# LiChaiUSTC/Speech-enhancement-based-on-a-maximum-likelihood-criterion

Hardware: AMD Instinct MI355X
Metric: training frames/sec (128-frame minibatch) (higher is better)
Workload: dtype f32

## Files before the change

include/mlggd.h:

```cpp
#ifndef MLGGD_H
#define MLGGD_H

#include <stddef.h>
#include <stdint.h>

#ifdef __cplusplus
extern "C" {
#endif

#define MLGGD_MAXLAYER 10
#define MLGGD_MAXCACHEFRAME 200000
#define MLGGD_UNIQUE_ID_BYTES 128
#define MLGGD_MAX_BETAS 32

enum {
    MLGGD_OK = 0,
    MLGGD_ERR_ARG = 1,
    MLGGD_ERR_DEVICE = 2,
    MLGGD_ERR_COMM = 3,
    MLGGD_ERR_STATE = 4
};

typedef struct mlggd_engine *mlggd_handle;

// ... 117 lines not shown

int mlggd_profile_select(mlggd_handle h, const char *kernel_class, int layer, int max_launches);
int mlggd_profile_stride(mlggd_handle h, int every_nth_step);
int mlggd_profile_read(mlggd_handle h, float *mean_usec, int *launches);
int mlggd_profile_overhead(mlggd_handle h, float *usec);
int mlggd_kernel_work(mlggd_handle h, const char *kernel_class, int layer, double *flops, double *bytes);
int mlggd_dw_launches_per_step(mlggd_handle h, int *launches);
int mlggd_dp_mode(mlggd_handle h, int *mode);
int mlggd_debug_fake_world(mlggd_handle h, int world_size, int mode);
int mlggd_debug_keep_ranks(mlggd_handle h, int on);
int mlggd_debug_rank_tensor(mlggd_handle h, const char *name, int layer, int rank, float *dst, size_t count);
int mlggd_debug_plan_count(mlggd_handle h, int *plans);

int mlggd_debug_out_slabs(mlggd_handle h, int *slabs);
int mlggd_debug_gemm_plan(mlggd_handle h, int layer, int *fwd_waves, int *dx_waves);

int mlggd_debug_math(mlggd_handle h, const char *fn, const float *x, float y, float *out, size_t n);

int mlggd_debug_stamp_select(mlggd_handle h, const char *kernel_class, int layer);
int mlggd_debug_stamp_read(mlggd_handle h, long long *out , int cap_blocks, int *blocks);

#ifdef __cplusplus
}
#endif
#endif
```

speech-enhancement-based-on-a-maximum-likelihood-criterion_amd/__init__.py:

```python
import collections
import ctypes as C
import os
import subprocess

import numpy as np

_HERE = os.path.dirname(os.path.abspath(__file__))
_CSRC = os.path.join(_HERE, "csrc")
LIB_PATH = os.path.join(_CSRC, "libmlggd.so")
MAXLAYER = 10
UNIQUE_ID_BYTES = 128

_fp = C.POINTER(C.c_float)
_fpp = C.POINTER(_fp)


class MlggdError(RuntimeError):
    pass


class _Config(C.Structure):
    _fields_ = [
        ("struct_size", C.c_int32), ("random_seed", C.c_int32), ("device", C.c_int32),
        ("numlayers", C.c_int32), ("layersizes", C.c_int32 * MAXLAYER), ("bunchsize", C.c_int32),
# ... 4 lines not shown
    ]


EXPORTS = [
    "mlggd_create", "mlggd_destroy", "mlggd_last_error", "mlggd_device_count", "mlggd_train_chunk",
    "mlggd_load_chunk", "mlggd_train_resident", "mlggd_sync", "mlggd_cv_sqerr", "mlggd_cv_abserr",
    "mlggd_cv_loglik", "mlggd_cv_all", "mlggd_forward", "mlggd_get_weights", "mlggd_set_weights",
    "mlggd_get_scalefactor", "mlggd_set_scalefactor", "mlggd_set_lrate", "mlggd_gamma",
    "mlggd_debug_tensor", "mlggd_comm_unique_id", "mlggd_comm_init", "mlggd_last_train_ms",
    "mlggd_profile_select", "mlggd_profile_stride", "mlggd_profile_read", "mlggd_profile_overhead",
    "mlggd_kernel_work", "mlggd_dw_launches_per_step", "mlggd_dp_mode", "mlggd_debug_fake_world",
    "mlggd_debug_stamp_select", "mlggd_debug_stamp_read",
    "mlggd_load_frames", "mlggd_train_frames", "mlggd_train_frames_async", "mlggd_cv_all_frames", "mlggd_forward_frames",
    "mlggd_alloc_pinned", "mlggd_alloc_pinned_on", "mlggd_free_pinned", "mlggd_set_cv_device_reduce",
    "mlggd_comm_info", "mlggd_debug_plan_count", "mlggd_debug_math", "mlggd_debug_out_slabs", "mlggd_debug_gemm_plan",
    "mlggd_debug_keep_ranks", "mlggd_debug_rank_tensor",
    "mlggd_wave_to_lps", "mlggd_lps_to_wave", "mlggd_enhance_wave",
    "mlggd_enhance_waves_layout", "mlggd_enhance_waves",
    "mlggd_score_waves", "mlggd_enhance_waves_scored",
    "mlggd_stoi_layout", "mlggd_stoi_waves", "mlggd_enhance_waves_scored_stoi",
    "mlggd_live_layout", "mlggd_live_open", "mlggd_live_push", "mlggd_live_received", "mlggd_live_close",
    "mlggd_error_stats", "mlggd_error_stats_frames", "mlggd_ggd_fit",
]
MAX_BETAS = 32

_lib = None


def build(force=False):
    srcs = [os.path.join(_CSRC, f) for f in ("engine.hip", "kernels.hip.h", "kernels64.hip.h", "spectral.hip.h", "score.hip.h", "live.hip.h",
# ... 42 lines not shown
    L.mlggd_profile_select.argtypes = [C.c_void_p, C.c_char_p, C.c_int, C.c_int]
    L.mlggd_profile_stride.argtypes = [C.c_void_p, C.c_int]
    L.mlggd_profile_read.argtypes = [C.c_void_p, _fp, C.POINTER(C.c_int)]
    L.mlggd_profile_overhead.argtypes = [C.c_void_p, _fp]
    L.mlggd_kernel_work.argtypes = [C.c_void_p, C.c_char_p, C.c_int, C.POINTER(C.c_double),
                                    C.POINTER(C.c_double)]
    L.mlggd_dw_launches_per_step.argtypes = [C.c_void_p, C.POINTER(C.c_int)]
    L.mlggd_dp_mode.argtypes = [C.c_void_p, C.POINTER(C.c_int)]
    L.mlggd_debug_fake_world.argtypes = [C.c_void_p, C.c_int, C.c_int]
    L.mlggd_debug_keep_ranks.argtypes = [C.c_void_p, C.c_int]
    L.mlggd_debug_rank_tensor.argtypes = [C.c_void_p, C.c_char_p, C.c_int, C.c_int, _fp, C.c_size_t]
    L.mlggd_comm_info.argtypes = [C.c_void_p, C.POINTER(C.c_int), C.POINTER(C.c_int)]
    L.mlggd_debug_plan_count.argtypes = [C.c_void_p, C.POINTER(C.c_int)]
    L.mlggd_debug_out_slabs.argtypes = [C.c_void_p, C.POINTER(C.c_int)]
    L.mlggd_debug_gemm_plan.argtypes = [C.c_void_p, C.c_int, C.POINTER(C.c_int), C.POINTER(C.c_int)]
    L.mlggd_debug_math.argtypes = [C.c_void_p, C.c_char_p, _fp, C.c_float, _fp, C.c_size_t]
    L.mlggd_debug_stamp_select.argtypes = [C.c_void_p, C.c_char_p, C.c_int]
    L.mlggd_debug_stamp_read.argtypes = [C.c_void_p, C.POINTER(C.c_longlong), C.c_int, C.POINTER(C.c_int)]
    _ip = C.POINTER(C.c_int32)
    L.mlggd_load_frames.argtypes = [C.c_void_p, C.c_int, C.c_int, _fp, _fp, C.c_int, _ip, C.c_int]
    L.mlggd_train_frames.argtypes = [C.c_void_p, C.c_int, C.c_int, _fp, _fp, C.c_int, _ip, C.c_int, C.POINTER(C.c_int)]
    L.mlggd_train_frames_async.argtypes = L.mlggd_train_frames.argtypes
    L.mlggd_cv_all_frames.argtypes = [C.c_void_p, C.c_int, C.c_int, _fp, _fp, C.c_int, _ip, C.c_int, _fp, _fp, _fp]
    L.mlggd_forward_frames.argtypes = [C.c_void_p, C.c_int, C.c_int, _fp, C.c_int, _ip, _fp]
    L.mlggd_alloc_pinned.argtypes = [C.c_size_t, C.POINTER(C.c_void_p)]
    L.mlggd_free_pinned.argtypes = [C.c_void_p]
    _sp = C.POINTER(C.c_int16)
    L.mlggd_wave_to_lps.argtypes = [C.c_int, C.c_int, C.c_int, _sp, C.POINTER(C.c_int), _fp]
    L.mlggd_lps_to_wave.argtypes = [C.c_int, C.c_int, C.c_int, _sp, C.c_int, _fp, _sp, _fp]
    L.mlggd_enhance_wave.argtypes = [C.c_void_p, C.c_int, C.c_int, _fp, _fp, C.c_int, _sp, _sp, _fp, C.POINTER(C.c_int)]
# ... 614 lines not shown
        return n.value

    def out_slabs(self):
        n = C.c_int(0)
        _check(load().mlggd_debug_out_slabs(self._h, C.byref(n)))
        return n.value

    def gemm_plan(self):
        out = []
        for l in range(1, len(self.layersizes)):
            f, d = C.c_int(0), C.c_int(0)
            _check(load().mlggd_debug_gemm_plan(self._h, l, C.byref(f), C.byref(d)))
            out.append((f.value, d.value))
        return out

    def comm_info(self):
        n, r = C.c_int(0), C.c_int(-1)
        _check(load().mlggd_comm_info(self._h, C.byref(n), C.byref(r)))
        return n.value, r.value

    def debug_math(self, fn, x, y=0.0):
        x = _f32(x).ravel()
        out = np.empty_like(x)
        _check(load().mlggd_debug_math(self._h, fn.encode(), _p(x), float(y), _p(out), x.size))
        return out

    def plan_count(self):
        n = C.c_int(0)
        _check(load().mlggd_debug_plan_count(self._h, C.byref(n)))
        return n.value
# ... 46 lines not shown
```

speech-enhancement-based-on-a-maximum-likelihood-criterion_amd/csrc/engine.hip:

```cpp
#include <hip/hip_runtime.h>
#include <hip/hip_ext.h>

#include <dlfcn.h>
#include <math.h>
#include <stdarg.h>
#include <stdio.h>
#include <stdlib.h>
#include <string.h>

#include <functional>
#include <mutex>
#include <string>
#include <vector>

#include "../../include/mlggd.h"
#include "kernels.hip.h"
#include "spectral.hip.h"
#include "score.hip.h"
#include "stoi.hip.h"
#include "stoi_rule.h"
#include "live.hip.h"
#include "live_rule.h"
#include "errstats.hip.h"

// ... 172 lines not shown
        WsBuf wave, lps, X, blk, out_i, out_f, lps_den, norm, frame_off, out_off, wave_off, utt_of;
        WsBuf clean, Xc, fstat, sframes, scores;
        WsBuf stoi_utt, stoi_x, stoi_f, stoi_i, stoi_res;
        std::vector<int32_t> h_frame_off, h_utt_of;
        std::vector<long long> h_out_off, h_wave_off;
        std::vector<float> h_norm;
        std::vector<float> h_scores;
        std::vector<StoiUtt> h_stoi_utt;
        std::vector<float> h_stoi;
        int lookup_table = 0;
    } ww;
    int live_groups = 0;
    bool indexed = false;
    int fdim = 0, toff = 0, raw_frames = 0;
    unsigned step_counter = 0;
    int fwd_pipe = 4, dx_pipe = 4;
    int tile64 = 1, n_cus = 256;
    int fwd_nw = 4, dx_nw = 4, dw_tile = 1, dw_persist = 1, dwp_per_cu = 2, dw_merge = 1, loss_fuse = 1, tile_map = 0, stage_ahead = 1;

    int world = 1, rank = 0;
    int dp_mode = 0;
    int shard_rows[MLGGD_MAXLAYER] = {0};
    int dp_a2a = 0;
    std::vector<float *> Ysrc[MLGGD_MAXLAYER];
    hipEvent_t ev_W[MLGGD_MAXLAYER] = {0}, ev_dw_done = nullptr;
    bool ev_W_pending[MLGGD_MAXLAYER] = {false};
    bool fake_world = false;
    float *Yall[MLGGD_MAXLAYER] = {0}, *dEdXall[MLGGD_MAXLAYER] = {0};
    bool keep_ranks = false;
    std::vector<float *> snap_x, snap_out, snap_y[MLGGD_MAXLAYER], snap_dedx[MLGGD_MAXLAYER];
    hipEvent_t ev_ready = nullptr, ev_gathered = nullptr;
// ... 223 lines not shown
    a.fdim = e->fdim;
    a.rows_out = rows_out;
    a.yblk = e->dp_a2a ? e->shard_rows[1] * 64 : 0;
    return a;
}
static int stage_blocks(const mlggd_engine *e) { return (e->lsp[0] / 32) * (e->Bp / 32); }
static float *in_bunch_other(mlggd_engine *e) {
    return e->in_bunch == e->in_bunch_buf[0] ? e->in_bunch_buf[1] : e->in_bunch_buf[0];
}

static bool tile64_ok(const mlggd_engine *e, int units_p) {
    if (e->tile64 == 0 || units_p % 64 != 0 || e->Bp % 64 != 0) return false;
    return e->tile64 == 2 || (long)(units_p / 64) * (e->Bp / 64) >= e->n_cus;
}
static bool fwd64_used(const mlggd_engine *e, int l) {
    if (e->fwd_pipe != 4 || e->fwd_nw != 4 || !tile64_ok(e, e->lsp[l])) return false;
    return l != e->L - 1 || e->S_out == 1;
}
static bool dx64_used(const mlggd_engine *e, int l) {
    return l >= 2 && e->dx_pipe == 4 && e->dx_nw == 4 && tile64_ok(e, e->lsp[l - 1]);
}

static int run_transpose(mlggd_engine *e, const Bunch &bn, int frames) {
    ProfScope ps(e, KC_TRANSPOSE, 0);
    hipLaunchKernelGGL(k_transpose_in, dim3(stage_blocks(e)), dim3(256), 0, e->stream,
                       stage_args(e, bn, frames, e->in_bunch));
    return launch_check("k_transpose_in");
}

static int wait_weight_gathers(mlggd_engine *e, int l_lo, int l_hi) {
    for (int l = l_lo; l <= l_hi; l++)
        if (e->ev_W_pending[l]) {
            HIPCHK(hipStreamWaitEvent(e->stream, e->ev_W[l], 0));
            e->ev_W_pending[l] = false;
        }
// ... 43 lines not shown
        const int Kp = e->lsp[l - 1], Np = e->lsp[l], n_tiles = Np / 32;
        CHK(wait_weight_gathers(e, l, l));
        if (cvscale) {
            const float keep = 1.0f - ((l == 1) ? e->cfg.visible_omit : e->cfg.hid_omit);
            hipLaunchKernelGGL(k_scale, dim3(1024), dim3(256), 0, e->stream, e->W[l], (size_t)Kp * Np, keep);
        }
        {
            if (((gather_flags & GATHER_HIDDEN_EACH) && l < e->L - 1) || ((gather_flags & GATHER_HIDDEN) && l == e->L - 2))
                gather_arm(e);
            ProfScope ps(e, KC_FWD, l);
            FwdArgs fa = fwd_args(e, l, e->Y[l]);
            if (fwd64_used(e, l)) {
                fa.n_tiles = Np / 64;
                fa.b_tiles = e->Bp / 64;
                fa.b_shift = log2_or_minus1(fa.b_tiles);
                const size_t lds = t64_lds_floats() * sizeof(float);
                if (l != e->L - 1) {
                    CHK(ensure_lds(e, k_fwd64<FWD_SIGMOID>, lds));
                    launch_timed(e, k_fwd64<FWD_SIGMOID>, dim3(fa.n_tiles * fa.b_tiles), dim3(256), lds, e->stream, fa);
                } else {
                    CHK(ensure_lds(e, k_fwd64<FWD_SLAB>, lds));
                    launch_timed(e, k_fwd64<FWD_SLAB>, dim3(fa.n_tiles * fa.b_tiles), dim3(256), lds, e->stream, fa);
                }
            } else if (l != e->L - 1) {
                long long *st = stamps_for(e, KC_FWD, l, n_tiles * b_tiles);
#define LAUNCH_FWD(NW, PIPE)                                                                                \
    {                                                                                                       \
        const size_t lds = fwd_lds_floats<NW, PIPE>() * sizeof(float);                                      \
        CHK(ensure_lds(e, k_fwd<FWD_SIGMOID, NW, PIPE>, lds));                                              \
        launch_timed(e, k_fwd<FWD_SIGMOID, NW, PIPE>, dim3(n_tiles * b_tiles), dim3(64 * NW), lds, e->stream, fa, st); \
    }
                if (e->fwd_nw == 16) LAUNCH_FWD(16, 0)
                else if (e->fwd_nw == 8 && e->fwd_pipe == 4) LAUNCH_FWD(8, 4)
                else if (e->fwd_nw == 8 && e->fwd_pipe) LAUNCH_FWD(8, 1)
                else if (e->fwd_nw == 8) LAUNCH_FWD(8, 0)
                else if (e->fwd_pipe == 4) LAUNCH_FWD(4, 4)
                else if (e->fwd_pipe) LAUNCH_FWD(4, 1)
                else LAUNCH_FWD(4, 0)
#undef LAUNCH_FWD
            } else {
                const int nwg = n_tiles * b_tiles * e->S_out;
                if (e->fwd_pipe == 4) {
                    const size_t lds = fwd_lds_floats<4, 4>() * sizeof(float);
                    CHK(ensure_lds(e, k_fwd<FWD_SLAB, 4, 4>, lds));
                    launch_timed(e, k_fwd<FWD_SLAB, 4, 4>, dim3(nwg), dim3(256), lds, e->stream, fa, (long long *)nullptr);
                } else {
                    const size_t lds = fwd_lds_floats<4, 1>() * sizeof(float);
                    launch_timed(e, k_fwd<FWD_SLAB, 4, 1>, dim3(nwg), dim3(256), lds, e->stream, fa, (long long *)nullptr);
                }
            }
        }
        CHK(launch_check("k_fwd"));
        if (cvscale) {
            const float keep = 1.0f - ((l == 1) ? e->cfg.visible_omit : e->cfg.hid_omit);
            hipLaunchKernelGGL(k_scale, dim3(1024), dim3(256), 0, e->stream, e->W[l], (size_t)Kp * Np, 1.0f / keep);
        }
        if (drop && l != e->L - 1) CHK(run_dropout(e, l, nullptr));
        if ((gather_flags & GATHER_HIDDEN_EACH) && l < e->L - 1) {
            CHK(gather_begin_armed(e));
            CHK(exchange_y(e, l, e->Y[l], nullptr));
            CHK(gather_end(e));
        }
// ... 451 lines not shown
    hipLaunchKernelGGL(k_loss_grad, dim3(n_loss), dim3(256), lds_grad, e->stream, e->eT, e->pT, colsum_in, B, e->D, e->Dp, Bp,
                       e->cfg.shapefactor, ML, nf, inv_n, e->scalefactor, e->dEdXt[L - 1], e->dEdX[L - 1], b_tiles);
    return launch_check("k_loss_grad");
}

static int run_dx(mlggd_engine *e, int l) {
    const int Kp = e->lsp[l - 1], b_tiles = e->Bp / 32;
    ProfScope ps(e, KC_DX, l);
    DxArgs xa = dx_args(e, l);
    if (dx64_used(e, l)) {
        xa.k_tiles = Kp / 64;
        xa.b_tiles = e->Bp / 64;
        xa.b_shift = log2_or_minus1(xa.b_tiles);
        const size_t lds = t64_lds_floats() * sizeof(float);
        CHK(ensure_lds(e, k_dx64, lds));
        launch_timed(e, k_dx64, dim3(xa.k_tiles * xa.b_tiles), dim3(256), lds, e->stream, xa);
        return launch_check("k_dx64");
    }
    long long *st = stamps_for(e, KC_DX, l, (Kp / 32) * b_tiles);
#define LAUNCH_DX(NW, PIPE)                                                                                  \
    {                                                                                                        \
        const size_t lds = dx_lds_floats<NW, PIPE>() * sizeof(float);                                        \
        CHK(ensure_lds(e, k_dx<NW, PIPE>, lds));                                                             \
        launch_timed(e, k_dx<NW, PIPE>, dim3((Kp / 32) * b_tiles), dim3(64 * NW), lds, e->stream, xa, st);      \
    }
    const bool dma = e->dx_pipe == 4 && (Kp / 32) * b_tiles <= 256;
    if (e->dx_nw == 8 && e->dx_pipe) LAUNCH_DX(8, 1)
    else if (e->dx_nw == 8) LAUNCH_DX(8, 0)
    else if (dma) LAUNCH_DX(4, 4)
    else if (e->dx_pipe) LAUNCH_DX(4, 1)
    else LAUNCH_DX(4, 0)
#undef LAUNCH_DX
    return launch_check("k_dx");
}

static int launch_dw_layer(mlggd_engine *e, int l, const float *in_rows, bool fused, float nf, hipStream_t st) {
    const int Kp = e->lsp[l - 1], Np = e->lsp[l];
    const long tiles128 = (long)((Kp + 127) / 128) * ((Np + 127) / 128);
    const bool big = e->dw_tile == 0 ? tiles128 >= 192 : e->dw_tile == 2;
    ProfScope ps(e, KC_DW, l, st);
    if (dwp_usable(e)) return launch_dwp(e, dwp_jobs(e, l, l, in_rows, nf), fused, st, l);
    if (big) return launch_dw<2>(e, l, in_rows, fused, nf, st);
    return launch_dw<1>(e, l, in_rows, fused, nf, st);
// ... 349 lines not shown
    e->device = cfg->device;
    for (int i = 0; i < e->L; i++) {
        e->ls[i] = cfg->layersizes[i];
        e->lsp[i] = ceil32(cfg->layersizes[i]);
    }
    e->B = cfg->bunchsize;
    e->Bp = ceil32(e->B);
    e->K0 = e->ls[0];
    e->D = e->ls[e->L - 1];
    e->Dp = e->lsp[e->L - 1];
    if (const char *v = getenv("MLGGD_FWD_NW")) e->fwd_nw = atoi(v);
    if (const char *v = getenv("MLGGD_WAVES_LOOKUP")) e->ww.lookup_table = !strcmp(v, "table");
    if (const char *v = getenv("MLGGD_DX_NW")) e->dx_nw = atoi(v);
    if (const char *v = getenv("MLGGD_FWD_PIPE")) e->fwd_pipe = atoi(v);
    if (const char *v = getenv("MLGGD_DX_PIPE")) e->dx_pipe = atoi(v);
    if (const char *v = getenv("MLGGD_DW_TILE")) e->dw_tile = atoi(v);
    if (const char *v = getenv("MLGGD_TWO_STREAMS")) e->two_streams = atoi(v);
    if (const char *v = getenv("MLGGD_DW_PERSIST")) e->dw_persist = atoi(v);
    if (const char *v = getenv("MLGGD_DWP_PER_CU")) e->dwp_per_cu = atoi(v);
    if (const char *v = getenv("MLGGD_DW_MERGE")) e->dw_merge = atoi(v);
    if (const char *v = getenv("MLGGD_LOSS_FUSE")) e->loss_fuse = atoi(v);
    if (const char *v = getenv("MLGGD_TILE_MAP")) e->tile_map = atoi(v);
    if (const char *v = getenv("MLGGD_STAGE_AHEAD")) e->stage_ahead = atoi(v);
    if (const char *v = getenv("MLGGD_CV_DEVICE")) e->cv_device = atoi(v) ? 1 : 0;
    if (const char *v = getenv("MLGGD_TILE64")) e->tile64 = atoi(v);
    *out = e;

    roctx_load();
    HIPCHK(hipSetDevice(e->device));
    {
// ... 943 lines not shown
    }
    if (nranks) *nranks = n;
    if (rank) *rank = r;
    return MLGGD_OK;
}
int mlggd_debug_plan_count(mlggd_handle e, int *plans) {
    if (!e || !plans) return fail(MLGGD_ERR_ARG, "NULL argument");
    *plans = (int)e->dwp_tables.size();
    return MLGGD_OK;
}
int mlggd_debug_gemm_plan(mlggd_handle e, int layer, int *fwd_waves, int *dx_waves) {
    if (!e || !fwd_waves || !dx_waves) return fail(MLGGD_ERR_ARG, "NULL argument");
    if (layer < 1 || layer >= e->L) return fail(MLGGD_ERR_ARG, "layer %d not in 1..%d", layer, e->L - 1);
    *fwd_waves = fwd64_used(e, layer) ? 1 : e->fwd_nw;
    *dx_waves = dx64_used(e, layer) ? 1 : e->dx_nw;
    return MLGGD_OK;
}
int mlggd_debug_out_slabs(mlggd_handle e, int *slabs) {
    if (!e || !slabs) return fail(MLGGD_ERR_ARG, "NULL argument");
    *slabs = e->S_out;
    return MLGGD_OK;
}
int mlggd_dp_mode(mlggd_handle e, int *mode) {
    if (!e || !mode) return fail(MLGGD_ERR_ARG, "NULL argument");
    *mode = (e->comm || e->fake_world) ? (e->dp_a2a ? 4 : 1 + e->dp_mode) : 0;
    return MLGGD_OK;
}

int mlggd_debug_math(mlggd_handle e, const char *fn, const float *x, float y, float *out, size_t n) {
    if (!e || !fn || (n > 0 && (!x || !out))) return fail(MLGGD_ERR_ARG, "NULL argument");
// ... 1230 lines not shown
```

speech-enhancement-based-on-a-maximum-likelihood-criterion_amd/csrc/kernels.hip.h:

```cpp
#pragma once
#include <hip/hip_runtime.h>

typedef float f32x16 __attribute__((ext_vector_type(16)));
typedef float f32x2 __attribute__((ext_vector_type(2)));

__device__ __forceinline__ f32x16 mfma32(float a, float b, f32x16 c) {
    return __builtin_amdgcn_mfma_f32_32x32x2f32(a, b, c, 0, 0, 0);
}
__device__ __forceinline__ int acc_row(int r, int lane) { return (r & 3) + 8 * (r >> 2) + 4 * (lane >> 5); }

__device__ __forceinline__ void divmod_by(int x, int d, int shift, int &q, int &r) {
    if (shift >= 0) {
        q = x >> shift;
        r = x & (d - 1);
    } else {
        q = (int)((unsigned)x / (unsigned)d);
        r = x - q * d;
    }
}
__device__ __forceinline__ void tile_of_block(int id, int u_tiles, int b_tiles, int b_shift, int &ut, int &bt, int map = 0) {
    if ((u_tiles & 7) == 0 && map != 2) {
        const int xcd = id & 7, slot = id >> 3;
        int q;
        divmod_by(slot, b_tiles, b_shift, q, bt);
// ... 144 lines not shown
}

enum { FWD_SIGMOID = 0, FWD_SLAB = 1 };

struct FwdArgs {
    const float *W, *Yt_in, *bias;
    float *Yt_out, *Y_out, *slab;
    int Kp, Np, Bp, N, n_tiles, b_tiles, S, map;
    int b_shift, s_shift;
    int yblk;
};
__device__ __forceinline__ size_t y_blocked_base(int u0, int yblk, int Bp) {
    const int blk = (int)((unsigned)u0 / (unsigned)yblk);
    return (size_t)blk * Bp * yblk + (u0 - blk * yblk);
}
template <int NW, int PIPE> constexpr int fwd_lds_floats() { return NW * (PIPE == 4 ? 4096 : 2048) + 32 * 36; }

template <int MODE, int NW, int PIPE = 1>
__device__ __forceinline__ void fwd_body(const FwdArgs &A, const int bid, float *smem, long long *stamps) {
    const float *__restrict__ W = A.W, *__restrict__ Yt_in = A.Yt_in, *__restrict__ bias = A.bias;
    float *__restrict__ Yt_out = A.Yt_out, *__restrict__ Y_out = A.Y_out, *__restrict__ slab = A.slab;
    const int Kp = A.Kp, Np = A.Np, Bp = A.Bp, N = A.N, n_tiles = A.n_tiles, b_tiles = A.b_tiles, S = A.S;
    float(*tileT)[36] = reinterpret_cast<float(*)[36]>(smem + NW * (PIPE == 4 ? 4096 : 2048));
    stamp(stamps, 0, bid);
    stamp_clk(stamps, 4, bid);
    const int tid = threadIdx.x, lane = tid & 63, wave = wave_id();
    const int i = lane & 31, h = lane >> 5;
    int id = bid, s = 0;
    if (MODE == FWD_SLAB) divmod_by(bid, S, A.s_shift, id, s);
    int nt, bt;
    tile_of_block(id, n_tiles, b_tiles, A.b_shift, nt, bt, A.map);
    const int n0 = nt * 32, b0 = bt * 32;

    const int P = Kp >> 1;
    const int slot = s * NW + wave, nslots = S * NW;
    int p0, p1;
    if (MODE == FWD_SLAB) {
        p0 = (int)((unsigned)(P * slot) / (unsigned)nslots);
// ... 3 lines not shown
        p1 = (int)((unsigned)(P * (wave + 1)) / (unsigned)NW);
    }
    const int npairs = p1 - p0;
    const int nch = (npairs + 15) >> 4;

    const rsrc_t rW = make_rsrc(W, (size_t)Kp * Np * 4), rY = make_rsrc(Yt_in, (size_t)Kp * Bp * 4);
    const int r8 = lane >> 3, c4 = lane & 7;
    const int voW = (r8 * Np + n0 + 4 * c4) * 4, voY = (r8 * Bp + b0 + 4 * c4) * 4;
    float *stg = smem + wave * 2048;
    float *wdst = stg + r8 * 32 + 4 * c4;
    const float *ard = stg + h * 32 + i, *brd = stg + 1024 + h * 32 + i;

    f32x16 acc;
#pragma unroll
    for (int r = 0; r < 16; r++) acc[r] = 0.0f;

    constexpr int NT_ = 64 * NW, EPT_ = 1024 / NT_ > 0 ? 1024 / NT_ : 1;
    static_assert(1024 % NT_ == 0, "every thread owns EPT_ whole output elements");
    float bias_pre[EPT_];
#pragma unroll
    for (int q = 0; q < EPT_; q++) bias_pre[q] = MODE == FWD_SIGMOID ? bias[n0 + ((tid + NT_ * q) >> 5)] : 0.0f;
    const float bias_row = (MODE == FWD_SIGMOID && NW == 4) ? bias[n0 + (tid >> 3)] : 0.0f;
    asm volatile("" ::: "memory");

    if constexpr (PIPE == 4) {
    float *t0 = smem + wave * 4096, *t1 = t0 + 2048;
    const int endW = Kp * Np * 4, endY = Kp * Bp * 4;
    float fa[16], fb[16], ga[16], gb[16];
#define FWD_DMA1(T, C, Q)                                                          \
    {                                                                              \
        const int row0 = 2 * (p0 + 16 * (C));                                      \
        const bool live = (C) < nch;                                               \
        __builtin_amdgcn_raw_ptr_buffer_load_lds(rW, (__attribute__((address_space(3))) void *)(T + (Q) * 256), 16, voW, \
                                                 live ? (row0 + 8 * (Q)) * Np * 4 : endW, 0, 0);        \
        __builtin_amdgcn_raw_ptr_buffer_load_lds(rY, (__attribute__((address_space(3))) void *)(T + 1024 + (Q) * 256), 16, voY, \
                                                 live ? (row0 + 8 * (Q)) * Bp * 4 : endY, 0, 0);        \
    }
#define FWD_RD4(T, NA, NB, Q)                                                      \
    {                                                                              \
// ... 168 lines not shown
            FWD_DRAIN(ga, gb, rem);
        } else {
            FWD_DRAIN(fa, fb, rem);
        }
    }
#undef FWD_LOAD1
#undef FWD_WRITE1
#undef FWD_READ4
#undef FWD_BODY
#undef FWD_DRAIN
    }

    stamp(stamps, 1, bid);
    __syncthreads();
    float(*red)[1024] = reinterpret_cast<float(*)[1024]>(smem);
#pragma unroll
    for (int r = 0; r < 16; r++) red[wave][acc_row(r, lane) * 32 + i] = acc[r];
    __syncthreads();
    stamp(stamps, 2, bid);
    if constexpr (NW == 4) {
        const int row = tid >> 3, col4 = (tid & 7) * 4;
        float4 v4 = *reinterpret_cast<const float4 *>(&red[0][row * 32 + col4]);
#pragma unroll
        for (int w = 1; w < NW; w++) {
            const float4 p4 = *reinterpret_cast<const float4 *>(&red[w][row * 32 + col4]);
            v4.x += p4.x;
            v4.y += p4.y;
            v4.z += p4.z;
            v4.w += p4.w;
        }
        if (MODE == FWD_SLAB) {
            *reinterpret_cast<float4 *>(&slab[((size_t)s * Np + n0 + row) * Bp + b0 + col4]) = v4;
// ... 51 lines not shown
            const int e = tid + NT * q, bl = e >> 5, nl = e & 31;
            if (e < 1024)
                Y_out[A.yblk ? y_blocked_base(n0, A.yblk, Bp) + (size_t)(b0 + bl) * A.yblk + nl : (size_t)(b0 + bl) * Np + n0 + nl] = tileT[bl][nl];
        }
    }
    stamp(stamps, 3, bid);
    stamp_clk(stamps, 6, bid);
}

#define DX_LDW 66
struct DxArgs {
    const float *W, *dEdXt, *Yt_prev;
    float *dEdXt_prev, *dEdX_prev;
    int Kp, Np, Bp, k_tiles, b_tiles, map, b_shift;
};
template <int NW, int PIPE> constexpr int dx_lds_floats() { return NW * (PIPE == 4 ? 8192 : 32 * DX_LDW + 2048) + 32 * 36; }

template <int NW, int PIPE = 1>
__device__ __forceinline__ void dx_body(const DxArgs &A, const int bid, float *smem, long long *stamps) {
    const float *__restrict__ W = A.W, *__restrict__ dEdXt = A.dEdXt, *__restrict__ Yt_prev = A.Yt_prev;
    float *__restrict__ dEdXt_prev = A.dEdXt_prev, *__restrict__ dEdX_prev = A.dEdX_prev;
    const int Kp = A.Kp, Np = A.Np, Bp = A.Bp, k_tiles = A.k_tiles, b_tiles = A.b_tiles;
    constexpr int WSZ = 32 * DX_LDW, STG = PIPE == 4 ? 8192 : WSZ + 2048;
    float(*tileT)[36] = reinterpret_cast<float(*)[36]>(smem + NW * STG);
    stamp(stamps, 0, bid);
    const int tid = threadIdx.x, lane = tid & 63, wave = wave_id();
    const int i = lane & 31, h = lane >> 5;
    int kt, bt;
    tile_of_block(bid, k_tiles, b_tiles, A.b_shift, kt, bt, A.map);
    const int k0 = kt * 32, b0 = bt * 32;

    const int Q = Np >> 2;
    const int qw = (Q + NW - 1) / NW;
    const int q0 = wave * qw;
    const int qend = (q0 + qw < Q) ? q0 + qw : Q;
    const int myq = qend > q0 ? qend - q0 : 0;
    const int nch = (myq + 15) >> 4;

// ... 1 lines not shown
    const rsrc_t rW = make_rsrc(W, (size_t)Kp * Np * 4), rD = make_rsrc(dEdXt, (size_t)Np * Bp * 4);
    const int wc4 = lane & 15, wr0 = lane >> 4;
    const int voW = ((k0 + wr0) * Np + 4 * wc4) * 4;
    const int r8 = lane >> 3, c4 = lane & 7;
    const int voD = (r8 * Bp + b0 + 4 * c4) * 4;
    const int wsw = (wc4 >= 8) ? 2 : 0;
    float *wdst = wb + wr0 * DX_LDW + 4 * wc4;
    float *ddst = db + ((r8 & ~3) | ((r8 & 1) << 1) | ((r8 >> 1) & 1)) * 32 + 4 * c4;
    const float *ard = wb + i * DX_LDW + 2 * h;
    const float *ard_hi = wb + i * DX_LDW + 2 * (1 - h);
    const float *brd = db + h * 32 + i;

    f32x16 acc;
#pragma unroll
    for (int r = 0; r < 16; r++) acc[r] = 0.0f;

    constexpr int NT_ = 64 * NW, EPT_ = 1024 / NT_ > 0 ? 1024 / NT_ : 1;
    static_assert(1024 % NT_ == 0, "every thread owns EPT_ whole output elements");
    float y_pre[EPT_];
    float4 y_pre4 = make_float4(0.0f, 0.0f, 0.0f, 0.0f);
    if constexpr (NW == 4) {
        y_pre4 = *reinterpret_cast<const float4 *>(&Yt_prev[(size_t)(k0 + (tid >> 3)) * Bp + b0 + (tid & 7) * 4]);
    } else {
#pragma unroll
        for (int q = 0; q < EPT_; q++) {
            const int e_ = tid + NT_ * q;
            y_pre[q] = Yt_prev[(size_t)(k0 + (e_ >> 5)) * Bp + b0 + (e_ & 31)];
        }
    }
    asm volatile("" ::: "memory");

    if constexpr (PIPE == 4) {
    float *ws0 = smem + wave * STG, *ds0 = ws0 + 2048, *ws1 = ws0 + 4096, *ds1 = ws0 + 6144;
    const int endW = Kp * Np * 4, endD = Np * Bp * 4;
    const int wr = lane >> 4, wq = lane & 15;
    int voWd[4];
#pragma unroll
    for (int tt = 0; tt < 4; tt++) voWd[tt] = ((k0 + wr) * Np + 4 * (wq ^ (4 * tt + wr))) * 4;
    const int voDd = (((r8 & ~3) | ((r8 & 1) << 1) | ((r8 >> 1) & 1)) * Bp + b0 + 4 * c4) * 4;
    int aoff[16];
#pragma unroll
    for (int j = 0; j < 16; j++) aoff[j] = i * 64 + 4 * (j ^ (i & 15)) + 2 * h;
    const int boff = h * 32 + i;
    float fa[32], fb[32], ga[32], gb[32];
#define DX_DMA1(WS, DS, C, T)                                                              \
    {                                                                                      \
// ... 189 lines not shown
            DX_DRAIN(ga, gb, rem);
        } else {
            DX_DRAIN(fa, fb, rem);
        }
    }
#undef DX_LOAD1
#undef DX_WRITE1
#undef DX_READ1
#undef DX_BODY
#undef DX_DRAIN
    }

    stamp(stamps, 1, bid);
    __syncthreads();
    float(*red)[1024] = reinterpret_cast<float(*)[1024]>(smem);
#pragma unroll
    for (int r = 0; r < 16; r++) red[wave][acc_row(r, lane) * 32 + i] = acc[r];
    __syncthreads();
    stamp(stamps, 2, bid);
    if constexpr (NW == 4) {
        const int row = tid >> 3, col4 = (tid & 7) * 4;
        float4 d4 = *reinterpret_cast<const float4 *>(&red[0][row * 32 + col4]);
#pragma unroll
        for (int w = 1; w < NW; w++) {
            const float4 p4 = *reinterpret_cast<const float4 *>(&red[w][row * 32 + col4]);
            d4.x += p4.x;
            d4.y += p4.y;
            d4.z += p4.z;
            d4.w += p4.w;
        }
        float4 g4;
        g4.x = (1.0f - y_pre4.x) * y_pre4.x * d4.x;
// ... 1101 lines not shown
```

Before: 1.004 million.

## Add 16x16x4 MFMA pipelined forward and dx GEMM variants as default

Adds a PIPE==16 form of the forward and dx GEMM kernels. It computes each 32x32 tile as four 16x16x4 f32 MFMAs instead of one 32x32x2 MFMA, with new swizzled LDS offsets and the same double-buffered buffer-to-LDS DMA scheme. This path becomes the default for non-64-tile layers, aiming for better MFMA throughput and latency hiding. It adds a debug query for which GEMM form each layer used, and it carries register-pressure and correctness risk from the new layouts.

```diff
diff --git a/include/mlggd.h b/include/mlggd.h
--- a/include/mlggd.h
+++ b/include/mlggd.h
@@ -155,6 +155,7 @@
 
 int mlggd_debug_out_slabs(mlggd_handle h, int *slabs);
 int mlggd_debug_gemm_plan(mlggd_handle h, int layer, int *fwd_waves, int *dx_waves);
+int mlggd_debug_gemm_form(mlggd_handle h, int layer, int *fwd_form, int *dx_form);
 
 int mlggd_debug_math(mlggd_handle h, const char *fn, const float *x, float y, float *out, size_t n);
 
diff --git a/speech-enhancement-based-on-a-maximum-likelihood-criterion_amd/__init__.py b/speech-enhancement-based-on-a-maximum-likelihood-criterion_amd/__init__.py
--- a/speech-enhancement-based-on-a-maximum-likelihood-criterion_amd/__init__.py
+++ b/speech-enhancement-based-on-a-maximum-likelihood-criterion_amd/__init__.py
@@ -42,6 +42,7 @@
     "mlggd_load_frames", "mlggd_train_frames", "mlggd_train_frames_async", "mlggd_cv_all_frames", "mlggd_forward_frames",
     "mlggd_alloc_pinned", "mlggd_alloc_pinned_on", "mlggd_free_pinned", "mlggd_set_cv_device_reduce",
     "mlggd_comm_info", "mlggd_debug_plan_count", "mlggd_debug_math", "mlggd_debug_out_slabs", "mlggd_debug_gemm_plan",
+    "mlggd_debug_gemm_form",
     "mlggd_debug_keep_ranks", "mlggd_debug_rank_tensor",
     "mlggd_wave_to_lps", "mlggd_lps_to_wave", "mlggd_enhance_wave",
     "mlggd_enhance_waves_layout", "mlggd_enhance_waves",
@@ -114,6 +115,7 @@
     L.mlggd_debug_plan_count.argtypes = [C.c_void_p, C.POINTER(C.c_int)]
     L.mlggd_debug_out_slabs.argtypes = [C.c_void_p, C.POINTER(C.c_int)]
     L.mlggd_debug_gemm_plan.argtypes = [C.c_void_p, C.c_int, C.POINTER(C.c_int), C.POINTER(C.c_int)]
+    L.mlggd_debug_gemm_form.argtypes = L.mlggd_debug_gemm_plan.argtypes
     L.mlggd_debug_math.argtypes = [C.c_void_p, C.c_char_p, _fp, C.c_float, _fp, C.c_size_t]
     L.mlggd_debug_stamp_select.argtypes = [C.c_void_p, C.c_char_p, C.c_int]
     L.mlggd_debug_stamp_read.argtypes = [C.c_void_p, C.POINTER(C.c_longlong), C.c_int, C.POINTER(C.c_int)]
@@ -758,6 +760,14 @@
             out.append((f.value, d.value))
         return out
 
+    def gemm_form(self):
+        out = []
+        for l in range(1, len(self.layersizes)):
+            f, d = C.c_int(0), C.c_int(0)
+            _check(load().mlggd_debug_gemm_form(self._h, l, C.byref(f), C.byref(d)))
+            out.append((f.value, d.value))
+        return out
+
     def comm_info(self):
         n, r = C.c_int(0), C.c_int(-1)
         _check(load().mlggd_comm_info(self._h, C.byref(n), C.byref(r)))
diff --git a/speech-enhancement-based-on-a-maximum-likelihood-criterion_amd/csrc/engine.hip b/speech-enhancement-based-on-a-maximum-likelihood-criterion_amd/csrc/engine.hip
--- a/speech-enhancement-based-on-a-maximum-likelihood-criterion_amd/csrc/engine.hip
+++ b/speech-enhancement-based-on-a-maximum-likelihood-criterion_amd/csrc/engine.hip
@@ -210,7 +210,8 @@
     bool indexed = false;
     int fdim = 0, toff = 0, raw_frames = 0;
     unsigned step_counter = 0;
-    int fwd_pipe = 4, dx_pipe = 4;
+    int fwd_pipe = 16, dx_pipe = 16;
+    int fwd_form[MLGGD_MAXLAYER], dx_form[MLGGD_MAXLAYER];
     int tile64 = 1, n_cus = 256;
     int fwd_nw = 4, dx_nw = 4, dw_tile = 1, dw_persist = 1, dwp_per_cu = 2, dw_merge = 1, loss_fuse = 1, tile_map = 0, stage_ahead = 1;
 
@@ -464,11 +465,11 @@
     return e->tile64 == 2 || (long)(units_p / 64) * (e->Bp / 64) >= e->n_cus;
 }
 static bool fwd64_used(const mlggd_engine *e, int l) {
-    if (e->fwd_pipe != 4 || e->fwd_nw != 4 || !tile64_ok(e, e->lsp[l])) return false;
+    if (!pipe_is_dma(e->fwd_pipe) || e->fwd_nw != 4 || !tile64_ok(e, e->lsp[l])) return false;
     return l != e->L - 1 || e->S_out == 1;
 }
 static bool dx64_used(const mlggd_engine *e, int l) {
-    return l >= 2 && e->dx_pipe == 4 && e->dx_nw == 4 && tile64_ok(e, e->lsp[l - 1]);
+    return l >= 2 && pipe_is_dma(e->dx_pipe) && e->dx_nw == 4 && tile64_ok(e, e->lsp[l - 1]);
 }
 
 static int run_transpose(mlggd_engine *e, const Bunch &bn, int frames) {
@@ -542,6 +543,7 @@
                 fa.n_tiles = Np / 64;
                 fa.b_tiles = e->Bp / 64;
                 fa.b_shift = log2_or_minus1(fa.b_tiles);
+                e->fwd_form[l] = 64;
                 const size_t lds = t64_lds_floats() * sizeof(float);
                 if (l != e->L - 1) {
                     CHK(ensure_lds(e, k_fwd64<FWD_SIGMOID>, lds));
@@ -556,24 +558,33 @@
     {                                                                                                       \
         const size_t lds = fwd_lds_floats<NW, PIPE>() * sizeof(float);                                      \
         CHK(ensure_lds(e, k_fwd<FWD_SIGMOID, NW, PIPE>, lds));                                              \
+        e->fwd_form[l] = PIPE;                                                                              \
         launch_timed(e, k_fwd<FWD_SIGMOID, NW, PIPE>, dim3(n_tiles * b_tiles), dim3(64 * NW), lds, e->stream, fa, st); \
     }
                 if (e->fwd_nw == 16) LAUNCH_FWD(16, 0)
-                else if (e->fwd_nw == 8 && e->fwd_pipe == 4) LAUNCH_FWD(8, 4)
+                else if (e->fwd_nw == 8 && pipe_is_dma(e->fwd_pipe)) LAUNCH_FWD(8, 4)
                 else if (e->fwd_nw == 8 && e->fwd_pipe) LAUNCH_FWD(8, 1)
                 else if (e->fwd_nw == 8) LAUNCH_FWD(8, 0)
+                else if (e->fwd_pipe == 16) LAUNCH_FWD(4, 16)
                 else if (e->fwd_pipe == 4) LAUNCH_FWD(4, 4)
                 else if (e->fwd_pipe) LAUNCH_FWD(4, 1)
                 else LAUNCH_FWD(4, 0)
 #undef LAUNCH_FWD
             } else {
                 const int nwg = n_tiles * b_tiles * e->S_out;
-                if (e->fwd_pipe == 4) {
+                if (e->fwd_pipe == 16) {
+                    const size_t lds = fwd_lds_floats<4, 16>() * sizeof(float);
+                    CHK(ensure_lds(e, k_fwd<FWD_SLAB, 4, 16>, lds));
+                    e->fwd_form[l] = 16;
+                    launch_timed(e, k_fwd<FWD_SLAB, 4, 16>, dim3(nwg), dim3(256), lds, e->stream, fa, (long long *)nullptr);
+                } else if (e->fwd_pipe == 4) {
                     const size_t lds = fwd_lds_floats<4, 4>() * sizeof(float);
                     CHK(ensure_lds(e, k_fwd<FWD_SLAB, 4, 4>, lds));
+                    e->fwd_form[l] = 4;
                     launch_timed(e, k_fwd<FWD_SLAB, 4, 4>, dim3(nwg), dim3(256), lds, e->stream, fa, (long long *)nullptr);
                 } else {
                     const size_t lds = fwd_lds_floats<4, 1>() * sizeof(float);
+                    e->fwd_form[l] = 1;
                     launch_timed(e, k_fwd<FWD_SLAB, 4, 1>, dim3(nwg), dim3(256), lds, e->stream, fa, (long long *)nullptr);
                 }
             }
@@ -1055,6 +1066,7 @@
         xa.b_shift = log2_or_minus1(xa.b_tiles);
         const size_t lds = t64_lds_floats() * sizeof(float);
         CHK(ensure_lds(e, k_dx64, lds));
+        e->dx_form[l] = 64;
         launch_timed(e, k_dx64, dim3(xa.k_tiles * xa.b_tiles), dim3(256), lds, e->stream, xa);
         return launch_check("k_dx64");
     }
@@ -1063,11 +1075,13 @@
     {                                                                                                        \
         const size_t lds = dx_lds_floats<NW, PIPE>() * sizeof(float);                                        \
         CHK(ensure_lds(e, k_dx<NW, PIPE>, lds));                                                             \
+        e->dx_form[l] = PIPE;                                                                                \
         launch_timed(e, k_dx<NW, PIPE>, dim3((Kp / 32) * b_tiles), dim3(64 * NW), lds, e->stream, xa, st);      \
     }
-    const bool dma = e->dx_pipe == 4 && (Kp / 32) * b_tiles <= 256;
+    const bool dma = pipe_is_dma(e->dx_pipe) && (Kp / 32) * b_tiles <= 256;
     if (e->dx_nw == 8 && e->dx_pipe) LAUNCH_DX(8, 1)
     else if (e->dx_nw == 8) LAUNCH_DX(8, 0)
+    else if (dma && e->dx_pipe == 16) LAUNCH_DX(4, 16)
     else if (dma) LAUNCH_DX(4, 4)
     else if (e->dx_pipe) LAUNCH_DX(4, 1)
     else LAUNCH_DX(4, 0)
@@ -1447,6 +1461,7 @@
     if (const char *v = getenv("MLGGD_DX_NW")) e->dx_nw = atoi(v);
     if (const char *v = getenv("MLGGD_FWD_PIPE")) e->fwd_pipe = atoi(v);
     if (const char *v = getenv("MLGGD_DX_PIPE")) e->dx_pipe = atoi(v);
+    for (int l = 0; l < MLGGD_MAXLAYER; l++) e->fwd_form[l] = e->dx_form[l] = -1;
     if (const char *v = getenv("MLGGD_DW_TILE")) e->dw_tile = atoi(v);
     if (const char *v = getenv("MLGGD_TWO_STREAMS")) e->two_streams = atoi(v);
     if (const char *v = getenv("MLGGD_DW_PERSIST")) e->dw_persist = atoi(v);
@@ -2420,6 +2435,13 @@
     if (layer < 1 || layer >= e->L) return fail(MLGGD_ERR_ARG, "layer %d not in 1..%d", layer, e->L - 1);
     *fwd_waves = fwd64_used(e, layer) ? 1 : e->fwd_nw;
     *dx_waves = dx64_used(e, layer) ? 1 : e->dx_nw;
+    return MLGGD_OK;
+}
+int mlggd_debug_gemm_form(mlggd_handle e, int layer, int *fwd_form, int *dx_form) {
+    if (!e || !fwd_form || !dx_form) return fail(MLGGD_ERR_ARG, "NULL argument");
+    if (layer < 1 || layer >= e->L) return fail(MLGGD_ERR_ARG, "layer %d not in 1..%d", layer, e->L - 1);
+    *fwd_form = e->fwd_form[layer];
+    *dx_form = e->dx_form[layer];
     return MLGGD_OK;
 }
 int mlggd_debug_out_slabs(mlggd_handle e, int *slabs) {
diff --git a/speech-enhancement-based-on-a-maximum-likelihood-criterion_amd/csrc/kernels.hip.h b/speech-enhancement-based-on-a-maximum-likelihood-criterion_amd/csrc/kernels.hip.h
--- a/speech-enhancement-based-on-a-maximum-likelihood-criterion_amd/csrc/kernels.hip.h
+++ b/speech-enhancement-based-on-a-maximum-likelihood-criterion_amd/csrc/kernels.hip.h
@@ -8,6 +8,11 @@
     return __builtin_amdgcn_mfma_f32_32x32x2f32(a, b, c, 0, 0, 0);
 }
 __device__ __forceinline__ int acc_row(int r, int lane) { return (r & 3) + 8 * (r >> 2) + 4 * (lane >> 5); }
+typedef float f32x4 __attribute__((ext_vector_type(4)));
+__device__ __forceinline__ f32x4 mfma16(float a, float b, f32x4 c) {
+    return __builtin_amdgcn_mfma_f32_16x16x4f32(a, b, c, 0, 0, 0);
+}
+constexpr bool pipe_is_dma(int pipe) { return pipe == 4 || pipe == 16; }
 
 __device__ __forceinline__ void divmod_by(int x, int d, int shift, int &q, int &r) {
     if (shift >= 0) {
@@ -182,14 +187,14 @@
     const int blk = (int)((unsigned)u0 / (unsigned)yblk);
     return (size_t)blk * Bp * yblk + (u0 - blk * yblk);
 }
-template <int NW, int PIPE> constexpr int fwd_lds_floats() { return NW * (PIPE == 4 ? 4096 : 2048) + 32 * 36; }
+template <int NW, int PIPE> constexpr int fwd_lds_floats() { return NW * (pipe_is_dma(PIPE) ? 4096 : 2048) + 32 * 36; }
 
 template <int MODE, int NW, int PIPE = 1>
 __device__ __forceinline__ void fwd_body(const FwdArgs &A, const int bid, float *smem, long long *stamps) {
     const float *__restrict__ W = A.W, *__restrict__ Yt_in = A.Yt_in, *__restrict__ bias = A.bias;
     float *__restrict__ Yt_out = A.Yt_out, *__restrict__ Y_out = A.Y_out, *__restrict__ slab = A.slab;
     const int Kp = A.Kp, Np = A.Np, Bp = A.Bp, N = A.N, n_tiles = A.n_tiles, b_tiles = A.b_tiles, S = A.S;
-    float(*tileT)[36] = reinterpret_cast<float(*)[36]>(smem + NW * (PIPE == 4 ? 4096 : 2048));
+    float(*tileT)[36] = reinterpret_cast<float(*)[36]>(smem + NW * (pipe_is_dma(PIPE) ? 4096 : 2048));
     stamp(stamps, 0, bid);
     stamp_clk(stamps, 4, bid);
     const int tid = threadIdx.x, lane = tid & 63, wave = wave_id();
@@ -223,6 +228,9 @@
     f32x16 acc;
 #pragma unroll
     for (int r = 0; r < 16; r++) acc[r] = 0.0f;
+    f32x4 c16[4];
+#pragma unroll
+    for (int q = 0; q < 4; q++) c16[q] = f32x4{0.0f, 0.0f, 0.0f, 0.0f};
 
     constexpr int NT_ = 64 * NW, EPT_ = 1024 / NT_ > 0 ? 1024 / NT_ : 1;
     static_assert(1024 % NT_ == 0, "every thread owns EPT_ whole output elements");
@@ -232,6 +240,94 @@
     const float bias_row = (MODE == FWD_SIGMOID && NW == 4) ? bias[n0 + (tid >> 3)] : 0.0f;
     asm volatile("" ::: "memory");
 
+    if constexpr (PIPE == 16) {
+    float *t0 = smem + wave * 4096, *t1 = t0 + 2048;
+    const int endW = Kp * Np * 4, endY = Kp * Bp * 4;
+    const int m16 = lane & 15, g4 = lane >> 4;
+    const int c4s = c4 ^ ((r8 & 2) << 1);
+    const int voWs = (r8 * Np + n0 + 4 * c4s) * 4, voYs = (r8 * Bp + b0 + 4 * c4s) * 4;
+    const int off0 = g4 * 32 + (g4 >> 1) * 16 + m16, off1 = off0 ^ 16;
+    float fa[16], fb[16], ga[16], gb[16];
+#define FWD_DMA1(T, C, Q)                                                          \
+    {                                                                              \
+        const int row0 = 2 * (p0 + 16 * (C));                                      \
+        const bool live = (C) < nch;                                               \
+        __builtin_amdgcn_raw_ptr_buffer_load_lds(rW, (__attribute__((address_space(3))) void *)(T + (Q) * 256), 16, voWs, \
+                                                 live ? (row0 + 8 * (Q)) * Np * 4 : endW, 0, 0);        \
+        __builtin_amdgcn_raw_ptr_buffer_load_lds(rY, (__attribute__((address_space(3))) void *)(T + 1024 + (Q) * 256), 16, voYs, \
+                                                 live ? (row0 + 8 * (Q)) * Bp * 4 : endY, 0, 0);        \
+    }
+#define FWD_RDQ(T, NA, NB, Q)                                                      \
+    {                                                                              \
+        NA[2 * (Q)] = (T)[off0 + 128 * (Q)];                                       \
+        NA[2 * (Q) + 1] = (T)[off1 + 128 * (Q)];                                   \
+        NB[2 * (Q)] = (T)[1024 + off0 + 128 * (Q)];                                \
+        NB[2 * (Q) + 1] = (T)[1024 + off1 + 128 * (Q)];                            \
+    }
+#define FWD_MFMAQ(A0, A1, B0, B1)                                                  \
+    {                                                                              \
+        c16[0] = mfma16(A0, B0, c16[0]);                                           \
+        c16[1] = mfma16(A0, B1, c16[1]);                                           \
+        c16[2] = mfma16(A1, B0, c16[2]);                                           \
+        c16[3] = mfma16(A1, B1, c16[3]);                                           \
+    }
+#define FWD_BODYD(FA, FB, NA, NB, TC, TN, C)                                       \
+    {                                                                              \
+        __builtin_amdgcn_s_waitcnt(0xC07F);  \
+        _Pragma("unroll") for (int g = 0; g < 4; g++) {                            \
+            FWD_MFMAQ(FA[2 * g], FA[2 * g + 1], FB[2 * g], FB[2 * g + 1]);         \
+            FWD_DMA1(TC, (C) + 2, g);                                              \
+            __builtin_amdgcn_sched_barrier(0);                                     \
+        }                                                                          \
+        __builtin_amdgcn_s_waitcnt(0x0F70 | 8);  \
+        _Pragma("unroll") for (int g = 4; g < 8; g++) {                            \
+            FWD_MFMAQ(FA[2 * g], FA[2 * g + 1], FB[2 * g], FB[2 * g + 1]);         \
+            FWD_RDQ(TN, NA, NB, 2 * (g - 4));                                      \
+            FWD_RDQ(TN, NA, NB, 2 * (g - 4) + 1);                                  \
+            __builtin_amdgcn_sched_barrier(0);                                     \
+        }                                                                          \
+    }
+#define FWD_DRAIND(FA, FB, CNT)                                                    \
+    {                                                                              \
+        _Pragma("unroll") for (int t = 0; t < 8; t++) {                            \
+            if (2 * t + 1 < (CNT)) {                                               \
+                FWD_MFMAQ(FA[2 * t], FA[2 * t + 1], FB[2 * t], FB[2 * t + 1]);     \
+            } else if (2 * t < (CNT)) {                                            \
+                const float a0 = g4 < 2 ? FA[2 * t] : 0.0f, a1 = g4 < 2 ? FA[2 * t + 1] : 0.0f; \
+                const float b0_ = g4 < 2 ? FB[2 * t] : 0.0f, b1_ = g4 < 2 ? FB[2 * t + 1] : 0.0f; \
+                FWD_MFMAQ(a0, a1, b0_, b1_);                                       \
+            }                                                                      \
+        }                                                                          \
+    }
+    if (nch > 0) {
+        const int nfull = npairs >> 4, rem = npairs & 15;
+#pragma unroll
+        for (int q = 0; q < 4; q++) FWD_DMA1(t0, 0, q);
+#pragma unroll
+        for (int q = 0; q < 4; q++) FWD_DMA1(t1, 1, q);
+        __builtin_amdgcn_s_waitcnt(0x0F70 | 8);
+#pragma unroll
+        for (int q = 0; q < 8; q++) FWD_RDQ(t0, fa, fb, q);
+        __builtin_amdgcn_sched_barrier(0);
+        int c = 0;
+        for (; c + 1 < nfull; c += 2) {
+            FWD_BODYD(fa, fb, ga, gb, t0, t1, c);
+            FWD_BODYD(ga, gb, fa, fb, t1, t0, c + 1);
+        }
+        if (c < nfull) {
+            FWD_BODYD(fa, fb, ga, gb, t0, t1, c);
+            FWD_DRAIND(ga, gb, rem);
+        } else {
+            FWD_DRAIND(fa, fb, rem);
+        }
+        __builtin_amdgcn_s_waitcnt(0x0F70 | 0);
+    }
+#undef FWD_DMA1
+#undef FWD_RDQ
+#undef FWD_MFMAQ
+#undef FWD_BODYD
+#undef FWD_DRAIND
+    } else
     if constexpr (PIPE == 4) {
     float *t0 = smem + wave * 4096, *t1 = t0 + 2048;
     const int endW = Kp * Np * 4, endY = Kp * Bp * 4;
@@ -430,8 +526,16 @@
     stamp(stamps, 1, bid);
     __syncthreads();
     float(*red)[1024] = reinterpret_cast<float(*)[1024]>(smem);
-#pragma unroll
-    for (int r = 0; r < 16; r++) red[wave][acc_row(r, lane) * 32 + i] = acc[r];
+    if constexpr (PIPE == 16) {
+#pragma unroll
+        for (int q = 0; q < 4; q++)
+#pragma unroll
+            for (int r = 0; r < 4; r++)
+                red[wave][(16 * (q >> 1) + 4 * (lane >> 4) + r) * 32 + 16 * (q & 1) + (lane & 15)] = c16[q][r];
+    } else {
+#pragma unroll
+        for (int r = 0; r < 16; r++) red[wave][acc_row(r, lane) * 32 + i] = acc[r];
+    }
     __syncthreads();
     stamp(stamps, 2, bid);
     if constexpr (NW == 4) {
@@ -513,14 +617,14 @@
     float *dEdXt_prev, *dEdX_prev;
     int Kp, Np, Bp, k_tiles, b_tiles, map, b_shift;
 };
-template <int NW, int PIPE> constexpr int dx_lds_floats() { return NW * (PIPE == 4 ? 8192 : 32 * DX_LDW + 2048) + 32 * 36; }
+template <int NW, int PIPE> constexpr int dx_lds_floats() { return NW * (pipe_is_dma(PIPE) ? 8192 : 32 * DX_LDW + 2048) + 32 * 36; }
 
 template <int NW, int PIPE = 1>
 __device__ __forceinline__ void dx_body(const DxArgs &A, const int bid, float *smem, long long *stamps) {
     const float *__restrict__ W = A.W, *__restrict__ dEdXt = A.dEdXt, *__restrict__ Yt_prev = A.Yt_prev;
     float *__restrict__ dEdXt_prev = A.dEdXt_prev, *__restrict__ dEdX_prev = A.dEdX_prev;
     const int Kp = A.Kp, Np = A.Np, Bp = A.Bp, k_tiles = A.k_tiles, b_tiles = A.b_tiles;
-    constexpr int WSZ = 32 * DX_LDW, STG = PIPE == 4 ? 8192 : WSZ + 2048;
+    constexpr int WSZ = 32 * DX_LDW, STG = pipe_is_dma(PIPE) ? 8192 : WSZ + 2048;
     float(*tileT)[36] = reinterpret_cast<float(*)[36]>(smem + NW * STG);
     stamp(stamps, 0, bid);
     const int tid = threadIdx.x, lane = tid & 63, wave = wave_id();
@@ -552,6 +656,9 @@
     f32x16 acc;
 #pragma unroll
     for (int r = 0; r < 16; r++) acc[r] = 0.0f;
+    f32x4 c16[4];
+#pragma unroll
+    for (int q = 0; q < 4; q++) c16[q] = f32x4{0.0f, 0.0f, 0.0f, 0.0f};
 
     constexpr int NT_ = 64 * NW, EPT_ = 1024 / NT_ > 0 ? 1024 / NT_ : 1;
     static_assert(1024 % NT_ == 0, "every thread owns EPT_ whole output elements");
@@ -568,6 +675,95 @@
     }
     asm volatile("" ::: "memory");
 
+    if constexpr (PIPE == 16) {
+    float *ws0 = smem + wave * STG, *ds0 = ws0 + 2048, *ws1 = ws0 + 4096, *ds1 = ws0 + 6144;
+    const int endW = Kp * Np * 4, endD = Np * Bp * 4;
+    const int wr = lane >> 4, wq = lane & 15;
+    int voWd[4];
+#pragma unroll
+    for (int tt = 0; tt < 4; tt++) voWd[tt] = ((k0 + wr) * Np + 4 * (wq ^ (4 * tt + wr))) * 4;
+    const int voDd = (r8 * Bp + b0 + 4 * (c4 ^ ((r8 & 2) << 1))) * 4;
+    const int m16 = lane & 15, g4 = lane >> 4;
+    const int pg = ((g4 & 1) << 1) | (g4 >> 1);
+    int aoff[16];
+#pragma unroll
+    for (int j = 0; j < 16; j++) aoff[j] = m16 * 64 + 4 * (j ^ m16) + pg;
+    const int boff0 = pg * 32 + (pg >> 1) * 16 + m16, boff1 = boff0 ^ 16;
+    float fa[32], fb[32], ga[32], gb[32];
+#define DX_DMA1(WS, DS, C, T)                                                              \
+    {                                                                                      \
+        const int quad0 = q0 + (C)*16;                                                     \
+        const bool live = (C) < nch;                                                       \
+        __builtin_amdgcn_raw_ptr_buffer_load_lds(rW, (__attribute__((address_space(3))) void *)(WS + (T) * 256), 16, \
+                                                 voWd[(T) & 3], live ? quad0 * 16 + (T) * (16 * Np) : endW, 0, 0); \
+        __builtin_amdgcn_raw_ptr_buffer_load_lds(rD, (__attribute__((address_space(3))) void *)(DS + (T) * 256), 16, \
+                                                 voDd, live ? (4 * quad0 + 8 * (T)) * Bp * 4 : endD, 0, 0); \
+    }
+#define DX_RD1(WS, DS, NA, NB, J)                                                          \
+    {                                                                                      \
+        NA[2 * (J)] = (WS)[aoff[J]];                                                       \
+        NA[2 * (J) + 1] = (WS)[aoff[J] + 1024];                                            \
+        NB[2 * (J)] = (DS)[boff0 + 128 * (J)];                                             \
+        NB[2 * (J) + 1] = (DS)[boff1 + 128 * (J)];                                         \
+    }
+#define DX_MFMAQ(FA, FB, J)                                                                \
+    {                                                                                      \
+        c16[0] = mfma16(FA[2 * (J)], FB[2 * (J)], c16[0]);                                 \
+        c16[1] = mfma16(FA[2 * (J)], FB[2 * (J) + 1], c16[1]);                             \
+        c16[2] = mfma16(FA[2 * (J) + 1], FB[2 * (J)], c16[2]);                             \
+        c16[3] = mfma16(FA[2 * (J) + 1], FB[2 * (J) + 1], c16[3]);                         \
+    }
+#define DX_BODYD(FA, FB, NA, NB, WC, DC, WN, DN, C)                                        \
+    {                                                                                      \
+        __builtin_amdgcn_s_waitcnt(0xC07F);  \
+        _Pragma("unroll") for (int g = 0; g < 8; g++) {                                    \
+            DX_MFMAQ(FA, FB, g);                                                           \
+            DX_DMA1(WC, DC, (C) + 2, g);                                                   \
+            __builtin_amdgcn_sched_barrier(0);                                             \
+        }                                                                                  \
+        __builtin_amdgcn_s_waitcnt(0x4F70);  \
+        _Pragma("unroll") for (int g = 8; g < 16; g++) {                                   \
+            DX_MFMAQ(FA, FB, g);                                                           \
+            DX_RD1(WN, DN, NA, NB, 2 * (g - 8));                                           \
+            DX_RD1(WN, DN, NA, NB, 2 * (g - 8) + 1);                                       \
+            __builtin_amdgcn_sched_barrier(0);                                             \
+        }                                                                                  \
+    }
+#define DX_DRAIND(FA, FB, CNT)                                                             \
+    {                                                                                      \
+        _Pragma("unroll") for (int j = 0; j < 16; j++) {                                   \
+            if (j < (CNT)) DX_MFMAQ(FA, FB, j);                                            \
+        }                                                                                  \
+    }
+    if (nch > 0) {
+        const int nfull = myq >> 4, rem = myq & 15;
+#pragma unroll
+        for (int t = 0; t < 8; t++) DX_DMA1(ws0, ds0, 0, t);
+#pragma unroll
+        for (int t = 0; t < 8; t++) DX_DMA1(ws1, ds1, 1, t);
+        __builtin_amdgcn_s_waitcnt(0x4F70);
+#pragma unroll
+        for (int j = 0; j < 16; j++) DX_RD1(ws0, ds0, fa, fb, j);
+        __builtin_amdgcn_sched_barrier(0);
+        int c = 0;
+        for (; c + 1 < nfull; c += 2) {
+            DX_BODYD(fa, fb, ga, gb, ws0, ds0, ws1, ds1, c);
+            DX_BODYD(ga, gb, fa, fb, ws1, ds1, ws0, ds0, c + 1);
+        }
+        if (c < nfull) {
+            DX_BODYD(fa, fb, ga, gb, ws0, ds0, ws1, ds1, c);
+            DX_DRAIND(ga, gb, rem);
+        } else {
+            DX_DRAIND(fa, fb, rem);
+        }
+        __builtin_amdgcn_s_waitcnt(0x0F70);
+    }
+#undef DX_DMA1
+#undef DX_RD1
+#undef DX_MFMAQ
+#undef DX_BODYD
+#undef DX_DRAIND
+    } else
     if constexpr (PIPE == 4) {
     float *ws0 = smem + wave * STG, *ds0 = ws0 + 2048, *ws1 = ws0 + 4096, *ds1 = ws0 + 6144;
     const int endW = Kp * Np * 4, endD = Np * Bp * 4;
@@ -787,8 +983,16 @@
     stamp(stamps, 1, bid);
     __syncthreads();
     float(*red)[1024] = reinterpret_cast<float(*)[1024]>(smem);
-#pragma unroll
-    for (int r = 0; r < 16; r++) red[wave][acc_row(r, lane) * 32 + i] = acc[r];
+    if constexpr (PIPE == 16) {
+#pragma unroll
+        for (int q = 0; q < 4; q++)
+#pragma unroll
+            for (int r = 0; r < 4; r++)
+                red[wave][(16 * (q >> 1) + 4 * (lane >> 4) + r) * 32 + 16 * (q & 1) + (lane & 15)] = c16[q][r];
+    } else {
+#pragma unroll
+        for (int r = 0; r < 16; r++) red[wave][acc_row(r, lane) * 32 + i] = acc[r];
+    }
     __syncthreads();
     stamp(stamps, 2, bid);
     if constexpr (NW == 4) {
```

Measured after the change: 988,800. -1.5%, worse.
